# underactuated/HSLabs

Measured on AMD Instinct MI355X. Metric: batched control-loop steps/sec (hexapod.xml, 18-DoF) at 1/2/4/8 MI355X, higher is better.
Workload: dtype f64

## Files before the change

hslabs_amd/csrc/hs_capi.cpp:

```cpp
#include <hip/hip_runtime.h>

#include <algorithm>
#include <atomic>
#include <cmath>
#include <cstdio>
#include <cstdlib>
#include <cstring>
#include <fstream>
#include <mutex>
#include <string>
#include <vector>

#include "hs_internal.h"

namespace {

thread_local std::string g_err;

int fail(int code, const std::string& msg) {
  g_err = msg;
  return code;
}

}
// ... 252 lines not shown
    if (e != hipSuccess) return hip_fail(e, "hipEventRecord");
  }
  if (key_reduce) {
    hs_run_args r = c;
    r.best_key = a.best_key;
    r.accumulate = 1;
    const int le = k.launch_fused_reduce(r, cx.total_mass, cx.rollout_mass, nullptr, 0);
    if (le != 0) return hip_fail((hipError_t)le, "kernel launch (best key)");
  }
  return HS_OK;
}

std::atomic<int64_t> g_limb_launches{0};
std::atomic<int64_t> g_limb_tile_launches{0};
std::atomic<int64_t> g_limb_tile_plan_launches{0};
std::atomic<int64_t> g_limb_tile_loop_launches{0};
#define HS_ONLINE_MAX_H 64

bool env_switch(const char* name, bool on_by_default) {
  const char* e = getenv(name);
  if (!e) return on_by_default;
  return on_by_default ? e[0] != '0' : e[0] == '1';
}

enum class step_route {
  ROLLOUT,
  ONLINE_DEFER,
  LIMB_ONLINE,
  FUSED,
  LIMB_FUSED,
};
enum class run_entry { STEPS, CALLS, FORCES_CALLS };

step_route route(const launch_ctx& cx, const hs_run_args& a, run_entry entry) {
  const bool forces = entry == run_entry::FORCES_CALLS, f32 = a.precision == HS_PREC_F32;
  const auto limb_eligible = [&] {
    return env_switch("HS_LIMB", true) && cx.host->limb_lane_ok && a.solve_mode == HS_SOLVE_AUTO && !a.q &&
           (forces || (!a.x && !a.dq)) && (!f32 || (!forces && env_switch("HS_LIMB_F32", true)));
  };
  const bool table = cx.map.ktab_n > 0 && (!cx.map.wave_rollouts || cx.map.limb_rollouts);
  if (entry != run_entry::STEPS) return limb_eligible() && table ? step_route::LIMB_FUSED : step_route::FUSED;
  if (a.horizon > HS_ONLINE_MAX_H) return step_route::ROLLOUT;
  if (env_switch("HS_LIMB_ONLINE", false) && limb_eligible())
    return table ? step_route::LIMB_ONLINE : step_route::ONLINE_DEFER;
  if (env_switch("HS_ONLINE_DEFER", false) && a.solve_mode == HS_SOLVE_AUTO) return step_route::ONLINE_DEFER;
  return step_route::ROLLOUT;
}

#ifndef HS_LIMB_TILE_MIN_STEPS
#define HS_LIMB_TILE_MIN_STEPS 40
#endif
bool limb_tile(step_route rt, const hs_run_args& a, int32_t n) {
  if (rt != step_route::LIMB_FUSED || !env_switch("HS_LIMB_TILE", true)) return false;
  if (const char* e = getenv("HS_LIMB_TILE_MIN")) {
    char* end = nullptr;
    const long min_n = strtol(e, &end, 10);
    if (end != e && *end == '\0' && min_n >= 1) return n >= min_n;
  }
  const int32_t idle = HS_TILE_SLOTS * limb_tile_count(n) - n;
  return a.precision != HS_PREC_F32 && n >= HS_LIMB_TILE_MIN_STEPS && 32 * idle <= n;
}
int32_t limb_tile_plan_mode() {
  if (!env_switch("HS_LIMB_TILE_PLAN", true)) return 0;
  const char* e = getenv("HS_LIMB_TILE_PLAN");
  return e && e[0] == '2' ? 2 : 1;
}
#ifndef HS_LIMB_TILE_LOOP_TILES
#define HS_LIMB_TILE_LOOP_TILES 5
#endif
#ifndef HS_LIMB_TILE_LOOP_ROUNDS
#define HS_LIMB_TILE_LOOP_ROUNDS 4
#endif
constexpr int64_t HS_RESIDENT_LIMB_WAVES = 2048;
int32_t limb_tile_loop(const hs_run_args& a, int32_t n) {
  const int32_t nt = limb_tile_count(n);
  if (a.precision == HS_PREC_F32) return 1;
  if (const char* e = getenv("HS_LIMB_TILE_LOOP")) {
    char* end = nullptr;
    const long tl = strtol(e, &end, 10);
    if (end != e && *end == '\0' && tl >= 1) return (int32_t)std::min<long>(tl, HS_TILE_PLAN_STEPS);
  }
  return limb_tile_loop_rule(nt, a.n_rollouts, HS_LIMB_TILE_LOOP_TILES, HS_LIMB_TILE_LOOP_ROUNDS * HS_RESIDENT_LIMB_WAVES);
}

#ifndef HS_FUSED_WAVES
#define HS_FUSED_WAVES 524288
#endif
#ifndef HS_FUSED_MAX_STEPS
#define HS_FUSED_MAX_STEPS 256
#endif
#ifndef HS_FUSED_RESERVE_STEPS
#define HS_FUSED_RESERVE_STEPS 1024
#endif
int32_t fused_chunk(const hs::launch_map& mp) {
  return std::max(1, std::min(HS_FUSED_MAX_STEPS, HS_FUSED_WAVES / std::max(1, mp.n_waves)));
}

size_t fix_counts_bytes(int32_t n_counts) { return ((size_t)n_counts * sizeof(int32_t) + 255) / 256 * 256; }
size_t fix_bytes(int32_t n_counts, int32_t chunk, const hs::launch_map& mp) {
  return fix_counts_bytes(n_counts) + (size_t)chunk * mp.n_waves * 2 * 2 * sizeof(int32_t);
}
void fix_carve(void* fix, int32_t n_counts, hs::launch_map& mp) {
  mp.fix_count = (int32_t*)fix;
  mp.fix_n_counts = n_counts;
  mp.fix_items = (int32_t*)((char*)fix + fix_counts_bytes(n_counts));
}
// ... 1584 lines not shown
```

hslabs_amd/csrc/hs_kernels.hip:

```cpp
#include <hip/hip_runtime.h>

#include <cfloat>
#include <cstdint>
#include <type_traits>

#ifndef HS_REAL_IS_FLOAT
#define HS_REAL_IS_FLOAT 0
#endif
#include "hs_internal.h"
#include "hs_math.h"

namespace {

using namespace hsd;

#ifndef HS_CURVED_LDS
#define HS_CURVED_LDS HS_REAL_IS_FLOAT
#endif
#ifndef HS_PRELOAD
#define HS_PRELOAD (!HS_REAL_IS_FLOAT)
#endif
#ifndef HS_KTE_PRELOAD
#define HS_KTE_PRELOAD (!HS_REAL_IS_FLOAT)
#endif
// ... 3145 lines not shown
  if (a.n_rollouts <= 0 || mp.n_waves <= 0) return 0;
  hipStream_t st = (hipStream_t)a.stream;
  RolloutWS* ws = (RolloutWS*)workspace;
  for (int h = 0; h < a.horizon; h++) {
    hs_run_args ah = a;
    launch_map mh = mp;
    ah.k0 = a.k0 + h;
    ah.accumulate = (h == 0) ? a.accumulate : 1;
    if (h + 1 < a.horizon) ah.best_key = nullptr;
    mh.h_row = h;
    if (h > 0 && mp.setup_io != SETUP_COMPUTE) mh.setup_io = SETUP_LOAD;
    if (mp.max_parts <= 18) launch_nm<18>(d_topo, ah, ws, mh, st);
    else if (mp.max_parts <= 22) launch_nm<22>(d_topo, ah, ws, mh, st);
    else launch_nm<HS_NMAX>(d_topo, ah, ws, mh, st);
    hipError_t e = hipGetLastError();
    if (e != hipSuccess) return (int)e;
  }
  return 0;
}

static int launch_fused(const hs_topo* d_topo, const hs_run_args& a, void* workspace, const launch_map& mp) {
  if (a.n_rollouts <= 0 || mp.n_waves <= 0) return 0;
  hipStream_t st = (hipStream_t)a.stream;
  RolloutWS* ws = (RolloutWS*)workspace;
  if (mp.setup_only) {
    int R;
    const int units = prep_units(mp, a.n_rollouts, R);
    const int64_t blocks = prep_blocks(units, R, mp.ttab_n, mp.ktab_nl > 0 ? mp.ktab_nl : HS_LMAX);
    if (mp.wave_model)
      hipLaunchKernelGGL(hs_prep_kernel<true>, dim3((unsigned)blocks), dim3(WAVE * HS_PREP_WPB), 0, st, d_topo, a, ws, mp);
    else
      hipLaunchKernelGGL(hs_prep_kernel<false>, dim3((unsigned)blocks), dim3(WAVE * HS_PREP_WPB), 0, st, d_topo, a, ws, mp);
    return (int)hipGetLastError();
  }
  launch_map m = mp;
  m.fused_w = mp.setup_only ? 0 : mp.n_waves;
  m.n_waves = mp.setup_only ? mp.n_waves : mp.n_waves * mp.fused_n;
  if (mp.fix_mode == FIX_SOLVE) m.n_waves = a.solve_mode != HS_SOLVE_AUTO ? 2 * m.n_waves : (m.n_waves < 256 ? m.n_waves : 256);
  if (mp.fix_mode == FIX_SOLVE && mp.fix_reduce) m.n_waves = (a.n_rollouts + WAVE - 1) / WAVE;
  if (mp.max_parts <= 18) launch_nm<18>(d_topo, a, ws, m, st);
  else if (mp.max_parts <= 22) launch_nm<22>(d_topo, a, ws, m, st);
  else launch_nm<HS_NMAX>(d_topo, a, ws, m, st);
  return (int)hipGetLastError();
}

static int launch_limb(const hs_topo* d_topo, const hs_run_args& a, void* workspace, const launch_map& mp,
                       int32_t tile_plan, int32_t* tile_planned) {
  if (tile_planned) *tile_planned = 0;
  if (a.n_rollouts <= 0 || mp.fused_n <= 0) return 0;
  hipStream_t st = (hipStream_t)a.stream;
  RolloutWS* ws = (RolloutWS*)workspace;
  launch_map m = mp;
  m.fused_w = mp.limb_rollouts ? mp.limb_waves : (a.n_rollouts + LGR - 1) / LGR;
  const int vsteps = mp.limb_tile ? HS_TILE_SLOTS * limb_tile_count(mp.fused_n) : mp.fused_n;
  m.limb_tile_loop = mp.limb_tile_loop < 1 || mp.tau_in || HS_REAL_IS_FLOAT ? 1 : mp.limb_tile_loop;
  const int wsteps = mp.limb_tile ? HS_TILE_SLOTS * limb_tile_chunks(limb_tile_count(mp.fused_n), m.limb_tile_loop) : mp.fused_n;
  const dim3 grid((unsigned)((int64_t)m.fused_w * wsteps));
  const int nm = mp.max_parts <= 18 ? 18 : (mp.max_parts <= 22 ? 22 : HS_NMAX);
  limb_tile_plan_arg plan = {};
  if (mp.limb_tile && tile_plan && mp.fused_n <= HS_TILE_PLAN_STEPS && mp.fused_h >= 1 && a.n_t >= 1 && a.k0 >= 0 &&
      mp.fused_s0 >= 0) {
    const limb_tile_launch L = {mp.fused_n, mp.fused_s0, mp.fused_h, a.k0, a.n_t, mp.ktab_nl > 0 ? mp.ktab_nl : HS_LMAX};
    bool planned = true;
    if (tile_plan == 2) {
      int row[HS_TILE_PLAN_STEPS];
      limb_tile_rows(L, row);
      limb_tile_chain_fill(row, L.n, plan.step);
    } else {
      planned = limb_tile_plan(L, plan.step);
    }
    if (planned) plan.n_slots = vsteps;
    if (tile_planned) *tile_planned = planned;
  }
#define HS_LIMB_LAUNCH(NM_, FORCES_)                                                                                  \
  do {                                                                                                                \
    if (mp.limb_tile)                                                                                                 \
      hipLaunchKernelGGL((hs_limb_kernel<NM_, FORCES_, true, limb_tile_plan_arg>), grid, dim3(WAVE), 0, st, d_topo, a, ws, \
                         m, plan);                                                                                    \
    else                                                                                                              \
      hipLaunchKernelGGL((hs_limb_kernel<NM_, FORCES_, false>), grid, dim3(WAVE), 0, st, d_topo, a, ws, m);           \
  } while (0)
#define HS_LIMB_LAUNCH_NM(FORCES_)               \
  do {                                           \
    if (nm == 18) HS_LIMB_LAUNCH(18, FORCES_);   \
    else if (nm == 22) HS_LIMB_LAUNCH(22, FORCES_); \
    else HS_LIMB_LAUNCH(HS_NMAX, FORCES_);       \
  } while (0)
  if (mp.tau_in) HS_LIMB_LAUNCH_NM(true);
  else HS_LIMB_LAUNCH_NM(false);
#undef HS_LIMB_LAUNCH_NM
#undef HS_LIMB_LAUNCH
  return (int)hipGetLastError();
}

__global__ void hs_fused_reduce_kernel(hs_run_args a, real total_mass, const double* __restrict__ rollout_mass,
                                       const real* __restrict__ ws, int n_steps) {
  reduce_rollouts(a, total_mass, rollout_mass, ws, n_steps, reinterpret_cast<uint64_t*>(a.best_key), a.key_steps);
}

static int launch_fused_reduce(const hs_run_args& a, double total_mass, const double* rollout_mass,
                               const void* work_steps, int32_t n_steps) {
  if (a.n_rollouts <= 0 || !a.work_cot) return 0;
  hipLaunchKernelGGL(hs_fused_reduce_kernel, dim3((a.n_rollouts + 63) / 64), dim3(64), 0, (hipStream_t)a.stream, a,
                     (real)total_mass, rollout_mass, (const real*)work_steps, n_steps);
  return (int)hipGetLastError();
}

#if HS_REAL_IS_FLOAT
#define HS_KERNELS_TABLE kernels_f32
#else
#define HS_KERNELS_TABLE kernels_f64
#endif
#ifndef __HIP_DEVICE_COMPILE__
extern const kernels HS_KERNELS_TABLE = {general_workspace_bytes, launch_rollouts,     launch_fused,
                                         launch_limb,             launch_fused_reduce, limb_deferred};
#endif

}
```

hslabs_amd/csrc/hs_limb.h:

```cpp

#ifndef HS_LIMB_GROUP
#define HS_LIMB_GROUP HS_FUSED_GROUP
#endif
#ifndef HS_LIMB_WAVES
#define HS_LIMB_WAVES 2
#endif
#ifndef HS_LIMB_WAVES_F32
#define HS_LIMB_WAVES_F32 HS_LIMB_WAVES
#endif

constexpr int LG = 8;
constexpr int LGR = WAVE / LG;

__device__ unsigned long long g_limb_deferred;

template <int NM, bool FORCES = false>
struct LimbLds {
  real g[NM][6];
  real a[6];
  real wd[HS_NMAX];
  real p[FORCES ? NM : 1][3];
};

__device__ inline real grp_get(real v, int src) { return __shfl(v, src); }
// ... 246 lines not shown
      mp.fix_items[2 * it] = s_glob - mp.fused_s0;
      mp.fix_items[2 * it + 1] = b;
    }
    return;
  }
  real kv[27];
#pragma unroll
  for (int e = 0; e < 27; e++) {
    const real v = limb ? vl[e] : real(0);
    real s = real(0) + v;
    for (int k = 1; k < nl; k++) {
      const real prev = dpp_r<0x111>(s);
      if (l >= 1) s = prev + v;
    }
    const real tot = grp_get(s, gbase + nl - 1);
    const real dtv = (e < 21) ? real(0) : (e < 24 ? S.a[e - 21] : S.a[e - 21]);
    kv[e] = (e < 21) ? wtt_entry(e, ts, n) + tot : tot - dtv;
  }
  opaque_vals<27>(kv);
  if (l == 0) FDBG(1, kv[0], 33);
  real K[36], rd[6], lam[6];
#pragma unroll
  for (int r = 0; r < 6; r++) {
#pragma unroll
    for (int c = 0; c < 6; c++) K[6 * r + c] = (c <= r) ? kv[pk(r, c)] : real(0);
    lam[r] = kv[21 + r];
  }
  ldl_n<6>(K, real(0), rd);
  ldl_solve_n<6>(K, rd, lam);
  if (l == 0) FDBG(2, lam[0], 34);
  bool nan = false;
  real t[3] = {0, 0, 0};
  if (limb) {
    for (int k = 0; k < 3; k++) {
      real s = rb[k];
      for (int r = 0; r < 6; r++) s -= Ct[3 * r + k] * lam[r];
      t[k] = s;
    }
    ldl_solve_n<3>(Bl, rdB, t);
    FDBG(24 + dbg_f, t[0], 35);
    for (int k = 0; k < 3; k++) nan |= t[k] != t[k];
    const int f = T->link[L][2].foot;
    if (live && a.cf)
      for (int k = 0; k < 3; k++) outp(a.cf)[orow * mp.st_cf + 3 * f + k] = t[k];
  }
  if (live && a.cf)
    for (int c = 3 * T->nf + l; c < mp.st_cf; c += LG) outp(a.cf)[orow * mp.st_cf + c] = real(0);
  const bool any_nan = grp_any(nan, gbase), any_bad = grp_any(limb && bad, gbase);
  if (l == 0 && live && a.flags) a.flags[orow] = (any_nan ? HS_FLAG_NAN : 0u) | (any_bad ? HS_FLAG_UNREACH : 0u);
}
#undef FDBG


__device__ inline int nth_bit16(uint32_t m, int r) {
  int sel = 0, cnt = 0;
#pragma unroll
  for (int i = 0; i < 16; i++) {
    const int s = (m >> i) & 1;
    if (s && cnt == r) sel = i;
    cnt += s;
  }
  return sel;
}
static_assert(HS_LMAX < LG, "lane LG - 1 of a group must not be a limb lane (lane_push's idle target)");
__device__ inline real lane_push(real v, int dst) {
  if constexpr (sizeof(real) == 8) {
    const double d = (double)v;
    const int lo = __builtin_amdgcn_ds_permute(dst << 2, __double2loint(d));
    const int hi = __builtin_amdgcn_ds_permute(dst << 2, __double2hiint(d));
    return (real)__hiloint2double(hi, lo);
  } else {
    return (real)__int_as_float(__builtin_amdgcn_ds_permute(dst << 2, __float_as_int((float)v)));
  }
}

#ifdef HS_DBG
#define TDBG(slot, val, n)                                                                                       \
  do {                                                                                                           \
    if (HS_DBG == (n) && dbg_r >= 0 && (size_t)dbg_r * 32 + (slot) < (1u << 22)) g_dbg[(size_t)dbg_r * 32 + (slot)] = (double)(val); \
  } while (0)
#else
#define TDBG(slot, val, n) do {} while (0)
#endif

#ifdef HS_STAMPS
#undef HS_STAMP_GATE
#define HS_STAMP_GATE stamp_on
#endif
template <bool FORCES>
__device__ __attribute__((always_inline)) inline void limb_tile_kd(
    const hs_topo* T_, real (&outer)[36][LGR * HS_LMAX], hs_link (&links)[HS_LMAX][3], const RolloutWS& W, bool straight,
    const real* u, real v, int lane, int nl, bool limb, int L, bool live, int row0, const real* tv, const real* o,
    real inv, real dt, real (&g3)[3][6], real (&Jp)[3][3], real (&Jz)[3][3], real* fp, bool& contact, bool& own,
    real* gown, real* jvel, real (&Pc)[3][3], real* Pown, bool& bad, bool& big, int dbg_r, bool stamp_on) {
  (void)dbg_r;
  (void)stamp_on;
  const int grp = lane >> 3, l = lane & 7;
  const int rprev = __shfl(row0, (lane + WAVE - LG) & (WAVE - 1)), rnext = __shfl(row0, (lane + LG) & (WAVE - 1));
  const uint64_t lv = __ballot(live);
  const bool lprev = grp > 0 && ((lv >> ((lane - LG) & (WAVE - 1))) & 1);
  const bool lnext = grp < LGR - 1 && ((lv >> ((lane + LG) & (WAVE - 1))) & 1);
  const bool shm = live && lprev && rprev + 2 == row0;
  const bool shp = live && lnext && rnext == row0 + 2;
  uint32_t M = 0;
  {
    const uint64_t bm = __ballot(live && !shm), bp = __ballot(live && !shp);
#pragma unroll
    for (int g = 0; g < LGR; g++)
      M |= (uint32_t)((bm >> (LG * g)) & 1) << (2 * g) | (uint32_t)((bp >> (LG * g)) & 1) << (2 * g + 1);
  }
  const int nreq = __popc(M);
  const int nidle = LG - nl;
  const int E0 = (LGR * nidle) / nl;
  const int rqm = __popc(M & ((1u << (2 * grp)) - 1)), rqp = __popc(M & ((1u << (2 * grp + 1)) - 1));
  const int pm = shm || rqm < E0 ? 0 : 1 + (rqm - E0) / LGR, pp = shp || rqp < E0 ? 0 : 1 + (rqp - E0) / LGR;
  auto col = [](int ln) { return (ln >> 3) * HS_LMAX + (ln & 7); };
  real P[3][3], U[3][3];
  BodyS om, op, oc;
  own = limb && T_->limb_own_n[L] > 0;
  {
    int rq = 0, fL = L;
    bool extra = false;
    if (!limb) {
      const int j = grp * nidle + (l - nl);
      rq = j / nl;
      fL = j - rq * nl;
      extra = rq < E0 && rq < nreq;
      if (!extra) rq = 0, fL = 0;
    }
    const int bit = nth_bit16(M, rq), gr = bit >> 1, side = bit & 1;
    const int rr = __shfl(row0, gr * LG);
    const int frow = limb ? row0 + 2 : rr + 4 * side;
    const int dst = gr * LG + fL;
    const int dm = limb ? (shp ? lane + LG : -1) : (extra && side == 0 ? dst : -1);
    const int dp = limb ? (shm ? lane - LG : -1) : (extra && side == 1 ? dst : -1);
    BodyS ob;
#pragma unroll
    for (int j = 0; j < 3; j++) ob.P[j] = ob.U[j] = real(0);
    if (limb || extra) {
      const hs_topo* T = opaque_s(T_);
      const bool fown = T->limb_own_n[fL] > 0;
      const A34 J = limb_frame(T, fL, straight, fown, W, frow, u, W.t_tab[frow] * v, ob);
      const real* ja = W.ktab[frow][fL];
      real sq[3], cq[3];
#pragma unroll
      for (int kk = 0; kk < 3; kk++) sincos_k_small(ja[kk], &sq[kk], &cq[kk]);
      A34 Jv = J, H;
#pragma unroll
      for (int kk = 0; kk < 3; kk++)
        fk_link<true>(T, links[fL][kk], kk, Jv, H, sq[kk], cq[kk], P[kk], U[kk], Jp[kk], Jz[kk], fp, contact);
      if (dm >= 0) {
        const int c = col(dm);
#pragma unroll
        for (int kk = 0; kk < 3; kk++)
#pragma unroll
          for (int j = 0; j < 3; j++) {
            outer[3 * kk + j][c] = P[kk][j];
            outer[9 + 3 * kk + j][c] = U[kk][j];
          }
      }
      if (dp >= 0) {
        const int c = col(dp);
#pragma unroll
        for (int kk = 0; kk < 3; kk++)
#pragma unroll
          for (int j = 0; j < 3; j++) {
            outer[18 + 3 * kk + j][c] = P[kk][j];
            outer[27 + 3 * kk + j][c] = U[kk][j];
          }
      }
    }
    if (!limb) contact = false;
    oc = ob;
    if (!straight) {
#pragma unroll
      for (int j = 0; j < 6; j++) {
        const real val = j < 3 ? ob.P[j] : ob.U[j - 3];
        const real vm = lane_push(val, dm >= 0 ? dm : LG - 1), vp = lane_push(val, dp >= 0 ? dp : LG - 1);
        if (pm == 0) (j < 3 ? om.P[j] : om.U[j - 3]) = vm;
        if (pp == 0) (j < 3 ? op.P[j] : op.U[j - 3]) = vp;
      }
    }
  }
  STAMP(1);
  for (int base = E0, pass = 1; base < nreq; base += LGR, pass++) {
    const bool act = limb && base + grp < nreq;
    const int bit = nth_bit16(M, act ? base + grp : 0), gr = bit >> 1, side = bit & 1;
    const int frow = __shfl(row0, gr * LG) + 4 * side;
    const int dst = act ? gr * LG + L : -1;
    BodyS ob;
#pragma unroll
    for (int j = 0; j < 3; j++) ob.P[j] = ob.U[j] = real(0);
    __builtin_amdgcn_sched_barrier(0);
    if (act) {
      real P2[3][3], U2[3][3];
      bool nb = false;
      const hs_topo* T = opaque_s(T_);
      limb_outer(T, links[L], limb_frame(T, L, straight, own, W, frow, u, W.t_tab[frow] * v, ob), W.ktab[frow][L], P2, U2,
                 nb);
      const int c = col(dst), o0 = side ? 18 : 0;
#pragma unroll
      for (int kk = 0; kk < 3; kk++)
#pragma unroll
        for (int j = 0; j < 3; j++) {
          outer[o0 + 3 * kk + j][c] = P2[kk][j];
          outer[o0 + 9 + 3 * kk + j][c] = U2[kk][j];
        }
    }
    if (!straight) {
#pragma unroll
      for (int j = 0; j < 6; j++) {
        const real val = j < 3 ? ob.P[j] : ob.U[j - 3];
        const real vm = lane_push(val, act && side == 0 ? dst : LG - 1), vp = lane_push(val, act && side == 1 ? dst : LG - 1);
        if (pm == pass) (j < 3 ? om.P[j] : om.U[j - 3]) = vm;
        if (pp == pass) (j < 3 ? op.P[j] : op.U[j - 3]) = vp;
      }
    }
  }
  __builtin_amdgcn_sched_barrier(0);
  STAMP(2);
  wave_sync();
  if (limb) {
    const hs_topo* T = T_;
    if (own) {
      if (straight) {
        om = body_straight(W.kf.own[L][0], u, tv[0]);
        op = body_straight(W.kf.own[L][0], u, tv[4]);
      }
      part_dyn((real)T->mass[T->limb_own[L][0]], inv, om.P, oc.P, op.P, om.U, oc.U, op.U, gown);
      part_g(oc.P, o, gown);
      if constexpr (FORCES)
        for (int j = 0; j < 3; j++) Pown[j] = oc.P[j];
    }
    const int ol = grp * HS_LMAX + l;
#pragma unroll
    for (int kk = 0; kk < 3; kk++) {
      real* P0 = P[kk];
      real* U0 = U[kk];
      opaque_vals<3>(P0);
      if constexpr (FORCES)
// ... 61 lines not shown
    struct {
      real outer[36][LGR * HS_LMAX];
    } k;
    LimbLds<NM, FORCES> g[LGR];
  };
  hs_link tl[HS_LMAX][3];
  __device__ hs_link (&links())[HS_LMAX][3] { return tl; }
};
static_assert(sizeof(LimbShared<HS_NMAX, false, true>) <= 20480, "a looping wavefront's LDS: 8 per CU's 160 KB");

struct LimbHead {
  int lane;
  int rslot, b;
  bool live;
  bool straight;
  const RolloutWS* W;
  real u[3];
};

template <class P>
__device__ inline const P* opaque_u(const P* p) {
  using cptr = const __attribute__((address_space(4))) P*;
  cptr q = (cptr)p;
  asm volatile("" : "+s"(q));
  return (const P*)q;
}

template <class P>
__device__ inline const P& opaque_k(const P& r) {
  using kptr = const __attribute__((address_space(4))) P*;
  kptr q = (kptr)&r;
  asm volatile("" : "+s"(q));
  return *(const P*)q;
}

template <int NM, bool FORCES, bool TILE, bool LOOP, class... PLAN>
__device__ __attribute__((always_inline)) inline void limb_step(LimbShared<NM, FORCES, LOOP>& sh, const hs_topo* __restrict__ T,
                                                                const hs_run_args& a0, const hs::launch_map& mp0,
                                                                const LimbHead& h, int fstep, bool stamp_on,
                                                                const PLAN&... plan) {
  (void)stamp_on;
  STAMP(23);
  int lane = h.lane;
  if constexpr (LOOP) {
    asm volatile("" : "+v"(lane));
    T = opaque_u(T);
  }
  const int grp = lane >> 3, l = lane & 7, gbase = lane & ~7, rslot = h.rslot, b = h.b;
  const int nl = T->n_limbs, nmj = T->nmj;
  const bool limb = l < nl, tlane = l == LG - 1, straight = h.straight;
  const int L = limb ? l : 0;
  const real u[3] = {h.u[0], h.u[1], h.u[2]};
  bool live = h.live;
  if constexpr (TILE) {
    const int slot0 = HS_TILE_SLOTS * fstep, ls = limb_tile_plan_step(plan..., slot0 + grp, mp0.fused_n);
    live = ls >= 0;
    fstep = live ? ls : limb_tile_plan_step(plan..., slot0, mp0.fused_n);
  }
  const RolloutWS* Wp = h.W;
  if constexpr (LOOP) Wp = opaque_u(Wp);
  const RolloutWS& W = *Wp;
  const real dt = W.st.dt;
  const real v = W.st.v;
  const real inv = real(1) / (2 * dt);
  LimbLds<NM, FORCES>& S = sh.g[grp];
  const int ol = grp * HS_LMAX + (l < HS_LMAX ? l : 0);
  const int s_glob = mp0.fused_s0 + fstep, call = s_glob / mp0.fused_h;
  const int k0 = (int)(((int64_t)a0.k0 + (int64_t)call * mp0.fused_h) % a0.n_t) + s_glob % mp0.fused_h;
  const int row0 = k0 - mp0.ktab_lo;
  real tv[5];
#pragma unroll
  for (int k = 0; k < 5; k += 2) tv[k] = W.t_tab[row0 + k] * v;
  real o[3];
  const real com0[3] = {(real)T->node[0].com[0], (real)T->node[0].com[1], (real)T->node[0].com[2]};
  if (straight) {
    for (int i = 0; i < 3; i++) o[i] = fma(tv[2], u[i], W.kf.torso[i]);
  } else {
    mulp(load34r(W.ktor[row0 + 2] + 6), com0, o);
  }
#ifdef HS_DBG
  const int dbg_r = live ? b * a0.horizon + s_glob : -1;
#define LDBG(slot, val, n)                                                                                       \
  do {                                                                                                           \
    if (HS_DBG == (n) && dbg_r >= 0 && (size_t)dbg_r * 32 + (slot) < (1u << 22)) g_dbg[(size_t)dbg_r * 32 + (slot)] = (double)(val); \
  } while (0)
#else
#define LDBG(slot, val, n) do {} while (0)
#endif

  real g0[6];
  {
    BodyS tb[3];
#pragma unroll
    for (int k = 0; k < 3; k++) {
      if (straight) tb[k] = body_straight(W.kf.torso, u, tv[2 * k]);
      else tb[k] = body_frame(load34r(W.ktor[row0 + 2 * k] + 6), com0);
    }
    part_dyn((real)T->mass[0], inv, tb[0].P, tb[1].P, tb[2].P, tb[0].U, tb[1].U, tb[2].U, g0);
    part_g(tb[1].P, o, g0);
  }
  STAMP(0);
  real g3[3][6];
  real Jp[3][3], Jz[3][3], fp[3];
  bool contact = false;
  bool own = false;
  real gown[6];
  real jvel[3];
  real Pc[3][3], Pown[3];
  bool bad = false, big = false;
  const hs_topo* const T_ = T;
  if constexpr (TILE) {
    limb_tile_kd<FORCES>(T_, sh.k.outer, sh.links(), W, straight, u, v, lane, nl, limb, L, live, row0, tv, o, inv, dt, g3,
                         Jp, Jz, fp, contact, own, gown, jvel, Pc, Pown, bad, big, live ? b * a0.horizon + s_glob : -1,
                         stamp_on);
  } else if (limb) {
    const int row = row0;
    own = T->limb_own_n[L] > 0;
    BodyS om, op, oc;
    {
      real P[3][3], U[3][3];
      const hs_topo* Ts = opaque_s(T);
      limb_outer(Ts, sh.k.links[L], limb_frame(Ts, L, straight, own, W, row, u, tv[0], om), W.ktab[row][L], P, U, big);
#pragma unroll
      for (int kk = 0; kk < 3; kk++)
#pragma unroll
        for (int j = 0; j < 3; j++) {
          sh.k.outer[3 * kk + j][ol] = P[kk][j];
          sh.k.outer[9 + 3 * kk + j][ol] = U[kk][j];
        }
    }
    STAMP(1);
    __builtin_amdgcn_sched_barrier(0);
    {
      real P[3][3], U[3][3];
      const hs_topo* Ts = opaque_s(T);
      limb_outer(Ts, sh.k.links[L], limb_frame(Ts, L, straight, own, W, row + 4, u, tv[4], op), W.ktab[row + 4][L], P, U,
                 big);
#pragma unroll
      for (int kk = 0; kk < 3; kk++)
#pragma unroll
        for (int j = 0; j < 3; j++) {
          sh.k.outer[18 + 3 * kk + j][ol] = P[kk][j];
          sh.k.outer[27 + 3 * kk + j][ol] = U[kk][j];
        }
    }
    __builtin_amdgcn_sched_barrier(0);
    STAMP(2);
    {
      const hs_topo* T = opaque_s(T_);
      const A34 J = limb_frame(T, L, straight, own, W, row + 2, u, tv[2], oc);
      if (own) {
        part_dyn((real)T->mass[T->limb_own[L][0]], inv, om.P, oc.P, op.P, om.U, oc.U, op.U, gown);
        part_g(oc.P, o, gown);
        if constexpr (FORCES)
          for (int j = 0; j < 3; j++) Pown[j] = oc.P[j];
      }
      const real* ja = W.ktab[row + 2][L];
      real sq[3], cq[3];
#pragma unroll
      for (int kk = 0; kk < 3; kk++) {
        big |= sincos_big(ja[kk]);
        sincos_k_small(ja[kk], &sq[kk], &cq[kk]);
      }
      A34 Jv = J, H;
#pragma unroll
      for (int kk = 0; kk < 3; kk++) {
        real P0[3], U0[3];
// ... 392 lines not shown
        for (int jj = 0; jj < 3; jj++)
          if (jj != r) s = s + cross_e(d, jj, r) * yy[jj];
        real xr = xt[kk][r] + s;
        tq = tq + Jz[kk][r] * xr;
      }
      real dw = tq * jvel[kk];
      S.wd[hh] = (dw > 0) ? dw : 0;
      nan |= tq != tq;
      if (live && a.tau) outp(a.tau)[orow * mp.st_tau + hh] = tq;
    }
    if (mine)
      for (int j = 0; j < 3; j++) nan |= y3[j] != y3[j];
    if (live && a.cf)
      for (int j = 0; j < 3; j++) {
        real zv = -real(0);
        if (mine) zv = -(real(0) + (real(-1)) * y3[j]);
        outp(a.cf)[orow * mp.st_cf + 3 * fiL + j] = zv;
      }
  }
  if (live && mp.limb_rollouts) {
    if (a.tau)
      for (int c = nmj + l; c < mp.st_tau; c += LG) outp(a.tau)[orow * mp.st_tau + c] = real(0);
    if (a.cf)
      for (int c = 3 * T->nf + l; c < mp.st_cf; c += LG) outp(a.cf)[orow * mp.st_cf + c] = real(0);
  }
  const bool any_nan = grp_any(nan, gbase), any_bad = grp_any(limb && bad, gbase);
  wave_sync();
  if (l == 0 && live) {
    uint32_t flags = 0;
    if (nc == 0) flags |= HS_FLAG_NO_CONTACT;
    if (nc == 1) flags |= HS_FLAG_FULL_RANK;
    if (nearf) flags |= HS_FLAG_NEAR_RANK;
    if (any_nan) flags |= HS_FLAG_NAN;
    if (any_bad) flags |= HS_FLAG_UNREACH;
    if (a.flags) a.flags[orow] = flags;
    real work_dt = real(0);
    for (int jj = 0; jj < nmj; jj++) work_dt += S.wd[jj];
    reinterpret_cast<real*>(mp.fused_work)[(size_t)s_glob * a.n_rollouts + b] = work_dt;
  }
  STAMP(9);
  RSTAMP(17);
}
#undef LDBG
#ifdef HS_STAMPS
#undef HS_STAMP_GATE
#define HS_STAMP_GATE true
#endif

struct LimbTileArgs {
  const hs_topo* T0;
  hs_run_args a;
  RolloutWS* rws;
  hs::launch_map mp;
  limb_tile_plan_arg plan;
};

template <int NM, bool FORCES, bool TILE = false, class... PLAN>
__global__ __launch_bounds__(WAVE, HS_REAL_IS_FLOAT ? HS_LIMB_WAVES_F32 : HS_LIMB_WAVES) void hs_limb_kernel(const hs_topo* __restrict__ T0, hs_run_args a,
                                                                      RolloutWS* __restrict__ rws, hs::launch_map mp, PLAN... plan) {
  static_assert(sizeof...(PLAN) == (TILE ? 1 : 0), "the tile mapping takes the launch's plan, the packed mapping nothing");
  static_assert(!TILE || (std::is_same<PLAN, limb_tile_plan_arg>::value && ...), "LimbTileArgs holds a limb_tile_plan_arg");
  static_assert(offsetof(LimbTileArgs, a) == 8 && offsetof(LimbTileArgs, rws) == 8 + sizeof(hs_run_args) &&
                    offsetof(LimbTileArgs, mp) == 16 + sizeof(hs_run_args) &&
                    offsetof(LimbTileArgs, plan) == 16 + sizeof(hs_run_args) + sizeof(hs::launch_map) &&
                    alignof(hs_run_args) == 8 && alignof(hs::launch_map) == 8,
                "LimbTileArgs: the kernel argument segment packs the arguments in order at their alignment");
  constexpr bool LOOP = TILE && !FORCES && !HS_REAL_IS_FLOAT;
  __shared__ LimbShared<NM, FORCES, LOOP> sh;
  int fstep = 0, q = (int)blockIdx.x;
  const int nt = TILE ? limb_tile_count(mp.fused_n) : 0, tl = LOOP ? mp.limb_tile_loop : 1;
  fused_coords<HS_LIMB_GROUP>((int)blockIdx.x, mp.fused_w, TILE ? HS_TILE_SLOTS * limb_tile_chunks(nt, tl) : mp.fused_n, fstep,
                              q);
  const hs_topo* __restrict__ T = mp.limb_model ? T0 + mp.limb_model[q] : T0;
  {
    const uint64_t* src = reinterpret_cast<const uint64_t*>(&T->link[0][0]);
    uint64_t* dst = reinterpret_cast<uint64_t*>(&sh.links()[0][0]);
    constexpr int NW = sizeof(hs_link[HS_LMAX][3]) / sizeof(uint64_t);
    for (int e = (int)threadIdx.x; e < NW; e += WAVE) dst[e] = src[e];
    wave_sync();
  }
  RSTAMP(16);
  STAMP(15);
  LimbHead h;
  h.lane = (int)threadIdx.x;
  h.rslot = q * LGR + (TILE ? fstep % LGR : h.lane >> 3);
  h.b = mp.limb_rollouts ? mp.limb_rollouts[h.rslot] : h.rslot;
  h.live = h.b >= 0 && h.b < a.n_rollouts;
  if (TILE && !h.live) return;
  const int bb = h.live ? h.b : (mp.limb_rollouts ? mp.limb_rollouts[q * LGR] : a.n_rollouts - 1);
  h.W = &rws[bb];
  const hs_gait_params& gp = a.params[bb];
  h.straight = (real)gp.curvature == 0 && !gp.rec_transform_flag;
  {
    const NodeK n0 = load_nodek(T, 0);
    for (int i = 0; i < 3; i++) h.u[i] = n0.Jp(i, 0);
  }
  if constexpr (LOOP) {
    const int c = fstep / LGR;
    for (int t0 = limb_tile_chunk_first(c, tl), t = t0, te = limb_tile_chunk_end(c, tl, nt); t < te; t++) {
      using kptr = const __attribute__((address_space(4))) LimbTileArgs*;
      kptr ka = (kptr)__builtin_amdgcn_kernarg_segment_ptr();
      asm volatile("" : "+s"(ka));
      const LimbTileArgs& k = *(const LimbTileArgs*)ka;
#ifdef HS_STAMPS
      const bool stamp_on = t - t0 == g_stamp_iter;
#else
      const bool stamp_on = true;
#endif
      limb_step<NM, FORCES, true, true>(sh, T, k.a, k.mp, h, t, stamp_on, k.plan);
      wave_sync();
    }
  } else {
    limb_step<NM, FORCES, TILE, false>(sh, T, a, mp, h, TILE ? fstep / LGR : fstep, true, plan...);
  }
// ... 2 lines not shown
```

hslabs_amd/csrc/hs_limb_tile.h:

```cpp
#pragma once

#include <stdint.h>

#if defined(__HIP__)
#define HS_TILE_FN __host__ __device__ inline
#else
#define HS_TILE_FN inline
#endif

constexpr int HS_TILE_SLOTS = 8;

HS_TILE_FN int limb_tile_count(int n) { return (n + HS_TILE_SLOTS - 1) / HS_TILE_SLOTS; }

HS_TILE_FN int limb_tile_step(int slot, int n) {
  const int n_even = (n + 1) / 2;
  if (slot < 0 || slot >= n) return -1;
  return slot < n_even ? 2 * slot : 2 * (slot - n_even) + 1;
}

HS_TILE_FN int limb_tile_chunks(int nt, int tl) {
  tl = tl < 1 ? 1 : tl;
  return (nt + tl - 1) / tl;
}
HS_TILE_FN int limb_tile_chunk_first(int c, int tl) { return c * (tl < 1 ? 1 : tl); }
// ... 89 lines not shown
    nxt[n_rem] = -1;
    if (tail[len] < 0) head[len] = n_rem;
    else nxt[tail[len]] = (int16_t)n_rem;
    tail[len] = n_rem++;
  };
  for (int i = 0; i < n; i++) {
    if (i >= 2 && row[i - 2] + 2 == row[i]) continue;
    int len = 1;
    while (i + 2 * len < n && row[i + 2 * len - 2] + 2 == row[i + 2 * len]) len++;
    const int full = len / HS_TILE_SLOTS * HS_TILE_SLOTS;
    for (int j = 0; j < full; j++) step[out++] = (int16_t)(i + 2 * j);
    if (len > full) push(i + 2 * full, len - full);
  }
  while (out < n) {
    int cap = n - out < HS_TILE_SLOTS ? n - out : HS_TILE_SLOTS;
    while (cap > 0) {
      int len = cap < HS_TILE_SLOTS - 1 ? cap : HS_TILE_SLOTS - 1;
      while (len > 0 && head[len] < 0) len--;
      int take = len;
      if (len == 0) {
        for (len = cap + 1; head[len] < 0; len++) {}
        take = cap;
      }
      const int r = head[len], first = rem0[r];
      head[len] = nxt[r];
      if (head[len] < 0) tail[len] = -1;
      for (int j = 0; j < take; j++) step[out++] = (int16_t)(first + 2 * j);
      if (len > take) push(first + 2 * take, len - take);
      cap -= take;
    }
  }
  for (; out < n_slots; out++) step[out] = -1;
}

HS_TILE_FN bool limb_tile_plan(const limb_tile_launch& L, int16_t* step, int* passes = nullptr,
                               int* parity_passes = nullptr) {
  if (L.n < 1 || L.n > HS_TILE_PLAN_STEPS || L.h < 1 || L.n_t < 1 || L.k0 < 0 || L.s0 < 0) return false;
  int16_t par[HS_TILE_PLAN_STEPS];
  int row[HS_TILE_PLAN_STEPS];
  limb_tile_rows(L, row);
  limb_tile_parity_fill(L.n, par);
  const int pp = limb_tile_passes(row, L.n, L.n_limbs, par);
  int pc = pp;
  if (pp > 0) {
    limb_tile_chain_fill(row, L.n, step);
    pc = limb_tile_passes(row, L.n, L.n_limbs, step);
  }
  if (parity_passes) *parity_passes = pp;
  if (passes) *passes = pc < pp ? pc : pp;
  if (pc < pp) return true;
  for (int s = 0; s < HS_TILE_SLOTS * limb_tile_count(L.n); s++) step[s] = par[s];
  return false;
}
```

Before: 982.1 million.

## Precompute per-tile slot rows and request masks on host in tile descriptor

The host now builds a per-tile descriptor for the limb tile path. Each tile carries its slot steps, table rows, the shared-neighbour request mask and a packed request list, and the whole descriptor is passed by value as a kernel argument. The kernel reads these instead of computing rows with modulo arithmetic, exchanging rows by shuffles, taking ballots to build the request mask and selecting the nth set bit in a loop. The cost is a larger kernel argument block, roughly 1.6 KB. The tile path is also restricted to launches whose rows fit in int16.

```diff
diff --git a/hslabs_amd/csrc/hs_capi.cpp b/hslabs_amd/csrc/hs_capi.cpp
--- a/hslabs_amd/csrc/hs_capi.cpp
+++ b/hslabs_amd/csrc/hs_capi.cpp
@@ -328,6 +328,7 @@
 #endif
 bool limb_tile(step_route rt, const hs_run_args& a, int32_t n) {
   if (rt != step_route::LIMB_FUSED || !env_switch("HS_LIMB_TILE", true)) return false;
+  if (!limb_tile_desc_ok(n, a.horizon, a.k0, a.n_t)) return false;
   if (const char* e = getenv("HS_LIMB_TILE_MIN")) {
     char* end = nullptr;
     const long min_n = strtol(e, &end, 10);
diff --git a/hslabs_amd/csrc/hs_kernels.hip b/hslabs_amd/csrc/hs_kernels.hip
--- a/hslabs_amd/csrc/hs_kernels.hip
+++ b/hslabs_amd/csrc/hs_kernels.hip
@@ -3221,30 +3221,33 @@
   RolloutWS* ws = (RolloutWS*)workspace;
   launch_map m = mp;
   m.fused_w = mp.limb_rollouts ? mp.limb_waves : (a.n_rollouts + LGR - 1) / LGR;
-  const int vsteps = mp.limb_tile ? HS_TILE_SLOTS * limb_tile_count(mp.fused_n) : mp.fused_n;
   m.limb_tile_loop = mp.limb_tile_loop < 1 || mp.tau_in || HS_REAL_IS_FLOAT ? 1 : mp.limb_tile_loop;
   const int wsteps = mp.limb_tile ? HS_TILE_SLOTS * limb_tile_chunks(limb_tile_count(mp.fused_n), m.limb_tile_loop) : mp.fused_n;
   const dim3 grid((unsigned)((int64_t)m.fused_w * wsteps));
   const int nm = mp.max_parts <= 18 ? 18 : (mp.max_parts <= 22 ? 22 : HS_NMAX);
-  limb_tile_plan_arg plan = {};
-  if (mp.limb_tile && tile_plan && mp.fused_n <= HS_TILE_PLAN_STEPS && mp.fused_h >= 1 && a.n_t >= 1 && a.k0 >= 0 &&
-      mp.fused_s0 >= 0) {
+  limb_tile_desc plan = {};
+  if (mp.limb_tile) {
     const limb_tile_launch L = {mp.fused_n, mp.fused_s0, mp.fused_h, a.k0, a.n_t, mp.ktab_nl > 0 ? mp.ktab_nl : HS_LMAX};
-    bool planned = true;
+    if (!limb_tile_desc_ok(L.n, L.h, L.k0, L.n_t) || L.s0 < 0) return (int)hipErrorInvalidValue;
+    int16_t step[HS_TILE_PLAN_STEPS];
+    bool planned = false;
     if (tile_plan == 2) {
       int row[HS_TILE_PLAN_STEPS];
       limb_tile_rows(L, row);
-      limb_tile_chain_fill(row, L.n, plan.step);
+      limb_tile_chain_fill(row, L.n, step);
+      planned = true;
+    } else if (tile_plan) {
+      planned = limb_tile_plan(L, step);
     } else {
-      planned = limb_tile_plan(L, plan.step);
-    }
-    if (planned) plan.n_slots = vsteps;
+      limb_tile_parity_fill(L.n, step);
+    }
+    if (!limb_tile_desc_fill(L, step, plan)) return (int)hipErrorInvalidValue;
     if (tile_planned) *tile_planned = planned;
   }
 #define HS_LIMB_LAUNCH(NM_, FORCES_)                                                                                  \
   do {                                                                                                                \
     if (mp.limb_tile)                                                                                                 \
-      hipLaunchKernelGGL((hs_limb_kernel<NM_, FORCES_, true, limb_tile_plan_arg>), grid, dim3(WAVE), 0, st, d_topo, a, ws, \
+      hipLaunchKernelGGL((hs_limb_kernel<NM_, FORCES_, true, limb_tile_desc>), grid, dim3(WAVE), 0, st, d_topo, a, ws, \
                          m, plan);                                                                                    \
     else                                                                                                              \
       hipLaunchKernelGGL((hs_limb_kernel<NM_, FORCES_, false>), grid, dim3(WAVE), 0, st, d_topo, a, ws, m);           \
diff --git a/hslabs_amd/csrc/hs_limb.h b/hslabs_amd/csrc/hs_limb.h
--- a/hslabs_amd/csrc/hs_limb.h
+++ b/hslabs_amd/csrc/hs_limb.h
@@ -322,16 +322,7 @@
 #undef FDBG
 
 
-__device__ inline int nth_bit16(uint32_t m, int r) {
-  int sel = 0, cnt = 0;
-#pragma unroll
-  for (int i = 0; i < 16; i++) {
-    const int s = (m >> i) & 1;
-    if (s && cnt == r) sel = i;
-    cnt += s;
-  }
-  return sel;
-}
+__device__ inline const limb_tile_entry& limb_tile_entry_of(const limb_tile_desc& d, int tile) { return d.tile[tile]; }
 static_assert(HS_LMAX < LG, "lane LG - 1 of a group must not be a limb lane (lane_push's idle target)");
 __device__ inline real lane_push(real v, int dst) {
   if constexpr (sizeof(real) == 8) {
@@ -360,26 +351,16 @@
 template <bool FORCES>
 __device__ __attribute__((always_inline)) inline void limb_tile_kd(
     const hs_topo* T_, real (&outer)[36][LGR * HS_LMAX], hs_link (&links)[HS_LMAX][3], const RolloutWS& W, bool straight,
-    const real* u, real v, int lane, int nl, bool limb, int L, bool live, int row0, const real* tv, const real* o,
-    real inv, real dt, real (&g3)[3][6], real (&Jp)[3][3], real (&Jz)[3][3], real* fp, bool& contact, bool& own,
+    const real* u, real v, int lane, int nl, bool limb, int L, bool live, int row0, uint32_t M, uint64_t req,
+    const real* tv, const real* o, real inv, real dt, real (&g3)[3][6], real (&Jp)[3][3], real (&Jz)[3][3], real* fp, bool& contact, bool& own,
     real* gown, real* jvel, real (&Pc)[3][3], real* Pown, bool& bad, bool& big, int dbg_r, bool stamp_on) {
   (void)dbg_r;
   (void)stamp_on;
   const int grp = lane >> 3, l = lane & 7;
-  const int rprev = __shfl(row0, (lane + WAVE - LG) & (WAVE - 1)), rnext = __shfl(row0, (lane + LG) & (WAVE - 1));
-  const uint64_t lv = __ballot(live);
-  const bool lprev = grp > 0 && ((lv >> ((lane - LG) & (WAVE - 1))) & 1);
-  const bool lnext = grp < LGR - 1 && ((lv >> ((lane + LG) & (WAVE - 1))) & 1);
-  const bool shm = live && lprev && rprev + 2 == row0;
-  const bool shp = live && lnext && rnext == row0 + 2;
-  uint32_t M = 0;
-  {
-    const uint64_t bm = __ballot(live && !shm), bp = __ballot(live && !shp);
-#pragma unroll
-    for (int g = 0; g < LGR; g++)
-      M |= (uint32_t)((bm >> (LG * g)) & 1) << (2 * g) | (uint32_t)((bp >> (LG * g)) & 1) << (2 * g + 1);
-  }
+  const bool shm = live && !((M >> (2 * grp)) & 1);
+  const bool shp = live && !((M >> (2 * grp + 1)) & 1);
   const int nreq = __popc(M);
+  auto nth_req = [req](int r) { return (int)(req >> (4 * r)) & 15; };
   const int nidle = LG - nl;
   const int E0 = (LGR * nidle) / nl;
   const int rqm = __popc(M & ((1u << (2 * grp)) - 1)), rqp = __popc(M & ((1u << (2 * grp + 1)) - 1));
@@ -398,7 +379,7 @@
       extra = rq < E0 && rq < nreq;
       if (!extra) rq = 0, fL = 0;
     }
-    const int bit = nth_bit16(M, rq), gr = bit >> 1, side = bit & 1;
+    const int bit = nth_req(rq), gr = bit >> 1, side = bit & 1;
     const int rr = __shfl(row0, gr * LG);
     const int frow = limb ? row0 + 2 : rr + 4 * side;
     const int dst = gr * LG + fL;
@@ -455,7 +436,7 @@
   STAMP(1);
   for (int base = E0, pass = 1; base < nreq; base += LGR, pass++) {
     const bool act = limb && base + grp < nreq;
-    const int bit = nth_bit16(M, act ? base + grp : 0), gr = bit >> 1, side = bit & 1;
+    const int bit = nth_req(act ? base + grp : 0), gr = bit >> 1, side = bit & 1;
     const int frow = __shfl(row0, gr * LG) + 4 * side;
     const int dst = act ? gr * LG + L : -1;
     BodyS ob;
@@ -623,10 +604,17 @@
   const int L = limb ? l : 0;
   const real u[3] = {h.u[0], h.u[1], h.u[2]};
   bool live = h.live;
+  int tile_row = 0;
+  uint32_t tile_M = 0;
+  uint64_t tile_req = 0;
   if constexpr (TILE) {
-    const int slot0 = HS_TILE_SLOTS * fstep, ls = limb_tile_plan_step(plan..., slot0 + grp, mp0.fused_n);
-    live = ls >= 0;
-    fstep = live ? ls : limb_tile_plan_step(plan..., slot0, mp0.fused_n);
+    const limb_tile_entry& te = limb_tile_entry_of(plan..., fstep);
+    const limb_tile_slot sl = te.slot[(unsigned)grp];
+    live = sl.step >= 0;
+    fstep = live ? sl.step : te.slot[0].step;
+    tile_row = sl.row;
+    tile_M = te.M;
+    tile_req = te.req;
   }
   const RolloutWS* Wp = h.W;
   if constexpr (LOOP) Wp = opaque_u(Wp);
@@ -636,8 +624,14 @@
   const real inv = real(1) / (2 * dt);
   LimbLds<NM, FORCES>& S = sh.g[grp];
   const int ol = grp * HS_LMAX + (l < HS_LMAX ? l : 0);
-  const int s_glob = mp0.fused_s0 + fstep, call = s_glob / mp0.fused_h;
-  const int k0 = (int)(((int64_t)a0.k0 + (int64_t)call * mp0.fused_h) % a0.n_t) + s_glob % mp0.fused_h;
+  const int s_glob = mp0.fused_s0 + fstep;
+  int k0;
+  if constexpr (TILE) {
+    k0 = tile_row;
+  } else {
+    const int call = s_glob / mp0.fused_h;
+    k0 = (int)(((int64_t)a0.k0 + (int64_t)call * mp0.fused_h) % a0.n_t) + s_glob % mp0.fused_h;
+  }
   const int row0 = k0 - mp0.ktab_lo;
   real tv[5];
 #pragma unroll
@@ -681,9 +675,9 @@
   bool bad = false, big = false;
   const hs_topo* const T_ = T;
   if constexpr (TILE) {
-    limb_tile_kd<FORCES>(T_, sh.k.outer, sh.links(), W, straight, u, v, lane, nl, limb, L, live, row0, tv, o, inv, dt, g3,
-                         Jp, Jz, fp, contact, own, gown, jvel, Pc, Pown, bad, big, live ? b * a0.horizon + s_glob : -1,
-                         stamp_on);
+    limb_tile_kd<FORCES>(T_, sh.k.outer, sh.links(), W, straight, u, v, lane, nl, limb, L, live, row0, tile_M, tile_req, tv,
+                         o, inv, dt, g3, Jp, Jz, fp, contact, own, gown, jvel, Pc, Pown, bad, big,
+                         live ? b * a0.horizon + s_glob : -1, stamp_on);
   } else if (limb) {
     const int row = row0;
     own = T->limb_own_n[L] > 0;
@@ -1182,14 +1176,14 @@
   hs_run_args a;
   RolloutWS* rws;
   hs::launch_map mp;
-  limb_tile_plan_arg plan;
+  limb_tile_desc plan;
 };
 
 template <int NM, bool FORCES, bool TILE = false, class... PLAN>
 __global__ __launch_bounds__(WAVE, HS_REAL_IS_FLOAT ? HS_LIMB_WAVES_F32 : HS_LIMB_WAVES) void hs_limb_kernel(const hs_topo* __restrict__ T0, hs_run_args a,
                                                                       RolloutWS* __restrict__ rws, hs::launch_map mp, PLAN... plan) {
-  static_assert(sizeof...(PLAN) == (TILE ? 1 : 0), "the tile mapping takes the launch's plan, the packed mapping nothing");
-  static_assert(!TILE || (std::is_same<PLAN, limb_tile_plan_arg>::value && ...), "LimbTileArgs holds a limb_tile_plan_arg");
+  static_assert(sizeof...(PLAN) == (TILE ? 1 : 0), "the tile mapping takes the launch's tile descriptor, the packed mapping nothing");
+  static_assert(!TILE || (std::is_same<PLAN, limb_tile_desc>::value && ...), "LimbTileArgs holds a limb_tile_desc");
   static_assert(offsetof(LimbTileArgs, a) == 8 && offsetof(LimbTileArgs, rws) == 8 + sizeof(hs_run_args) &&
                     offsetof(LimbTileArgs, mp) == 16 + sizeof(hs_run_args) &&
                     offsetof(LimbTileArgs, plan) == 16 + sizeof(hs_run_args) + sizeof(hs::launch_map) &&
diff --git a/hslabs_amd/csrc/hs_limb_tile.h b/hslabs_amd/csrc/hs_limb_tile.h
--- a/hslabs_amd/csrc/hs_limb_tile.h
+++ b/hslabs_amd/csrc/hs_limb_tile.h
@@ -165,3 +165,65 @@
   for (int s = 0; s < HS_TILE_SLOTS * limb_tile_count(L.n); s++) step[s] = par[s];
   return false;
 }
+
+constexpr int HS_TILE_DESC_TILES = HS_TILE_PLAN_STEPS / HS_TILE_SLOTS;
+
+struct alignas(4) limb_tile_slot {
+  int16_t step;
+  int16_t row;
+};
+struct limb_tile_entry {
+  limb_tile_slot slot[HS_TILE_SLOTS];
+  uint32_t M;
+  uint32_t nreq;
+  uint64_t req;
+};
+struct limb_tile_desc {
+  int32_t n_tiles;
+  int32_t pad_;
+  limb_tile_entry tile[HS_TILE_DESC_TILES];
+};
+static_assert(sizeof(limb_tile_entry) == 48, "a tile's descriptor: 8 slots of 4 bytes, M, nreq and the request list");
+static_assert(sizeof(limb_tile_desc) == 8 + 48 * HS_TILE_DESC_TILES && sizeof(limb_tile_desc) <= 1600,
+              "the descriptor travels by value: with the kernel's other arguments well under 4 KB");
+
+HS_TILE_FN bool limb_tile_desc_ok(int n, int h, int k0, int n_t) {
+  return n >= 1 && n <= HS_TILE_PLAN_STEPS && h >= 1 && n_t >= 1 && k0 >= 0 && (int64_t)n_t + h <= 32767;
+}
+
+HS_TILE_FN void limb_tile_entry_fill(const int* row, const int16_t* slots, limb_tile_entry& e) {
+  const int first = slots[0] >= 0 ? row[slots[0]] : 0;
+  uint32_t M = 0;
+  for (int g = 0; g < HS_TILE_SLOTS; g++) {
+    e.slot[g].step = (int16_t)(slots[g] >= 0 ? slots[g] : -1);
+    e.slot[g].row = (int16_t)(slots[g] >= 0 ? row[slots[g]] : first);
+    if (slots[g] < 0) continue;
+    const int r = row[slots[g]];
+    const bool shm = g > 0 && slots[g - 1] >= 0 && row[slots[g - 1]] + 2 == r;
+    const bool shp = g < HS_TILE_SLOTS - 1 && slots[g + 1] >= 0 && row[slots[g + 1]] == r + 2;
+    M |= (uint32_t)!shm << (2 * g) | (uint32_t)!shp << (2 * g + 1);
+  }
+  e.M = M;
+  e.nreq = 0;
+  e.req = 0;
+  for (int bit = 0; bit < 2 * HS_TILE_SLOTS; bit++)
+    if ((M >> bit) & 1) e.req |= (uint64_t)bit << (4 * e.nreq++);
+}
+
+HS_TILE_FN bool limb_tile_desc_fill(const limb_tile_launch& L, const int16_t* step, limb_tile_desc& d) {
+  if (!limb_tile_desc_ok(L.n, L.h, L.k0, L.n_t) || L.s0 < 0) return false;
+  int row[HS_TILE_PLAN_STEPS];
+  for (int i = 0; i < L.n; i++) row[i] = limb_tile_row(L, i);
+  d.n_tiles = limb_tile_count(L.n);
+  d.pad_ = 0;
+  for (int t = 0; t < HS_TILE_DESC_TILES; t++) {
+    if (t < d.n_tiles) {
+      limb_tile_entry_fill(row, step + HS_TILE_SLOTS * t, d.tile[t]);
+    } else {
+      for (int g = 0; g < HS_TILE_SLOTS; g++) d.tile[t].slot[g].step = -1, d.tile[t].slot[g].row = 0;
+      d.tile[t].M = d.tile[t].nreq = 0;
+      d.tile[t].req = 0;
+    }
+  }
+  return true;
+}
```

Result: faster. 1.038 billion, median of 6 (+5.7%).
